# Alan-404/Conformer

Hardware: AMD Instinct MI355X
Metric: encoder audio-frames/sec (B=32,T=1000,d=512,L=16) (higher is better)
Workload: dtype f32; 1 GPU; cfg2 Conformer-L Encoder.forward: B=32/GPU, T=1000 mel frames (T'=249), d=512, 16 blocks, 8 heads, k=31, fp32, eval, random-init weights, batch-sharded replicas; per_gpu_batch=32, mel_frames=1000

## Files before the change

### conformer_amd/_lib.py

```python
from __future__ import annotations

import ctypes
import os
from ctypes import c_char_p, c_float, c_int, c_int64, c_uint64, c_void_p

_HERE = os.path.dirname(os.path.abspath(__file__))
LIB_PATH = os.environ.get("CONFORMER_AMD_LIB") or os.path.join(_HERE, "lib", "libconformer_hip.so")

_P, _I, _L, _F, _U = c_void_p, c_int, c_int64, c_float, c_uint64
ABI_VERSION = 4

SIGNATURES = {
    "cfm_version": (c_int, []),
    "cfm_abi_version": (c_int, []),
    "cfm_gemm_bias_stats_f32": (c_int, [_P, _P, _P, _P, _P, _L, _I, _I, _L, _L, _P]),
    "cfm_gemm_bias_residual_stats_f32": (c_int, [_P, _P, _P, _P, _F, _P, _P, _L, _I, _I, _L, _L, _L, _P]),
    "cfm_gemm_splitk_f32": (c_int, [_I, _P, _P, _P, _P, _F, _P, _P, _I, _L, _I, _I, _L, _L, _L, _P]),
    "cfm_gemm_lnfold_f32": (c_int, [_I, _P, _P, _I, _F, _P, _P, _P, _P, _L, _I, _I, _L, _L, _P]),
    "cfm_layernorm_fwd_stats_f32": (c_int, [_P, _P, _P, _P, _P, _L, _I, _F, _P]),
    "cfm_ffn_pack_elems": (ctypes.c_int64, [_I, _I]),
    "cfm_ffn_pack_f32": (c_int, [_P, _P, _P, _I, _I, _P]),
    "cfm_rowgemm_pack_f32": (c_int, [_P, _P, _I, _I, _I, _P]),
    "cfm_rowchain_f32": (c_int, [_I, _I, _I, _I, _P, _L, _P, _P, _P, _L, _P, _L, _P, _I, _F, _P, _P, _P, _P, _F, _I, _P, _L, _P, _P, _P, _F,
                                 _P, _P, _P, _F, _P, _L, _L, _I, _P]),
# ... 83 lines not shown
    "cfm_hotword_pack": (c_int, [_I, _P, _P, _I, _P, _P, _I, _P, _P, _P, _P, ctypes.c_size_t]),
    "cfm_hotword_count": (c_int, [_P, _P, _P, _I, ctypes.c_double, _P, _P, _P]),
    "cfm_ctc_beam_hw_workspace_bytes": (ctypes.c_size_t, [_I, _I, _I, _I]),
    "cfm_ctc_beam_hw_decode_f32": (c_int, [_P, _P, _I, _I, _I, _I, _I, _I, _F, _F, _I, _P, ctypes.c_double, ctypes.c_double,
                                           ctypes.c_double, _I, _P, ctypes.c_double, _P, ctypes.c_size_t, _P, _P, _P, _P, _P,
                                           _P]),
    "cfm_ctc_beam_stream_state_bytes": (ctypes.c_size_t, [_I, _I, _I, _I, _I, _I]),
    "cfm_ctc_beam_stream_init": (c_int, [_I, _I, _I, _I, _P, _I, _P, _P, ctypes.c_size_t, _P]),
    "cfm_ctc_beam_stream_step_f32": (c_int, [_P, _P, _I, _I, _I, _I, _I, _I, _F, _F, _I, _P, ctypes.c_double, ctypes.c_double,
                                             ctypes.c_double, _I, _P, ctypes.c_double, _P, ctypes.c_size_t, _I, _I, _P, _P, _P,
                                             _P, _P, _P]),
    "cfm_ctc_beam_stream_finish_f32": (c_int, [_I, _I, _I, _I, _P, ctypes.c_double, ctypes.c_double, ctypes.c_double, _I, _P,
                                               ctypes.c_double, _P, ctypes.c_size_t, _I, _P, _P, _P, _P, _P, _P]),
    "cfm_ctc_beam_stream_reset_slots": (c_int, [_I, _I, _I, _I, _P, _I, _P, _P, _I, _P, ctypes.c_size_t, _P]),
    "cfm_lstm_fwd_carry_f32": (c_int, [_P, _P, _P, _P, _P, _P, _P, _P, _I, _I, _I, _P]),
    "cfm_lstm_fwd_frag_carry_f32": (c_int, [_P, _P, _P, _P, _P, _P, _P, _P, _P, _I, _I, _I, _P]),
    "cfm_lstm_fwd_mfma16_carry_f32": (c_int, [_I, _P, _P, _P, _P, _P, _P, _P, _P, _P, _I, _I, _I, _P]),
    "cfm_lstm_fwd_f32": (c_int, [_P, _P, _P, _P, _P, _P, _P, _I, _I, _I, _P]),
    "cfm_lstm_fwd_frag_f32": (c_int, [_P, _P, _P, _P, _P, _P, _P, _P, _I, _I, _I, _P]),
    "cfm_lstm_bwd_frag_f32": (c_int, [_P, _P, _P, _P, _P, _P, _P, _P, _I, _I, _I, _P]),
    "cfm_debug_lstm_trace": (c_int, [_P]),
    "cfm_debug_dw16_trace": (c_int, [_P]),
    "cfm_linear_bwd_weight_mfma16_f32": (c_int, [_I, _P, _I, _L, _P, _I, _L, _P, _L, _P, _I, _I, _L, _F, _P]),
    "cfm_lstm_fwd_mfma16_f32": (c_int, [_I, _P, _P, _P, _P, _P, _P, _P, _P, _I, _I, _I, _P]),
    "cfm_lstm_bwd_mfma16_f32": (c_int, [_I, _P, _P, _P, _P, _P, _P, _P, _P, _I, _I, _I, _P]),
    "cfm_lstm_bwd_f32": (c_int, [_P, _P, _P, _P, _P, _P, _P, _I, _I, _I, _P]),
    "cfm_swish_bn_eval_f32": (c_int, [_P, _P, _P, _P, _P, _F, _P, _L, _I, _P]),
    "cfm_swish_bn_stats_f32": (c_int, [_P, _P, _P, _P, _P, _F, _L, _I, _P]),
    "cfm_swish_bn_bwd_f32": (c_int, [_P, _P, _P, _P, _P, _F, _I, _P, _P, _P, _L, _I, _P]),
    "cfm_split_pack_elems": (ctypes.c_int64, [_I, _I, _I]),
    "cfm_split_pack_bf16_f32": (c_int, [_I, _P, _P, _I, _I, _P]),
    "cfm_gemm_split_bf16_f32": (c_int, [_I, _I, _P, _P, _P, _P, _F, _P, _L, _I, _I, _L, _L, _L, _P]),
    "cfm_subsample_conv2_relu_split_bf16_f32": (c_int, [_I, _P, _P, _P, _P, _I, _I, _I, _I, _P]),
    "cfm_ctc_workspace_floats": (ctypes.c_int64, [_I, _I, _I]),
    "cfm_ctc_loss_fwd_f32": (c_int, [_P, _P, _P, _L, _L, _P, _P, _I, _I, _I, _I, _I, _P, _P, _P]),
    "cfm_ctc_loss_bwd_f32": (c_int, [_P, _P, _P, _L, _L, _P, _P, _I, _I, _I, _I, _I, _P, _P, _P, _P]),
    "cfm_ctc_align_workspace_bytes": (ctypes.c_size_t, [_I, _I, _I]),
    "cfm_ctc_align_f32": (c_int, [_P, _P, _P, _P, _I, _I, _I, _I, _I, _P, ctypes.c_size_t, _P, _P, _P, _P, _P, _P, _P, _P]),
    "cfm_relpos_attention_rows_f32": (c_int, [_P, _P, _P, _L, _P, _L, _P, _P, _P, _P, _L, _I, _I, _I, _I, _I, _I, _I, _P, _P]),
    "cfm_relpos_attention_slots_f32": (c_int, [_P, _P, _P, _L, _P, _L, _P, _P, _P, _P, _P, _P, _L, _I, _I, _I, _I, _I, _I, _P, _P]),
    "cfm_relpos_attention_slots_mfma16_f32": (c_int, [_I, _P, _P, _P, _I, _L, _P, _L, _P, _P, _P, _P, _P, _P, _L, _I, _I, _I, _I, _I, _I,
                                                      _P, _P]),
    "cfm_debug_attention_trace_f32": (c_int, [_P, _P, _P, _L, _P, _L, _P, _P, _P, _P, _L, _I, _I, _I, _I, _P, _P]),
    "cfm_debug_set_bwd_tile": (c_int, [_I]),
    "cfm_debug_set_attention_waves": (c_int, [_I]),
    "cfm_debug_gemm_cfg_f32": (c_int, [_I, _P, _P, _P, _P, _F, _P, _L, _I, _I, _P, _P]),
    "cfm_debug_set_conv2_bk": (c_int, [_I]),
    "cfm_debug_ffn_trace": (c_int, [_P, _I]),
    "cfm_debug_ffn_variant": (c_int, [_I]),
    "cfm_debug_ffn_layout": (c_int, [_I, _I]),
    "cfm_relpos_table_f32": (c_int, [_P, _P, _I, _I, _P]),
    "cfm_relpos_attention_fwd_f32": (c_int, [_P, _P, _P, _L, _P, _L, _P, _P, _P, _P, _L, _P, _I, _I, _I, _I, _P]),
    "cfm_dwconv_bn_swish_fwd_f32": (c_int, [_P, _P, _P, _P, _P, _P, _P, _F, _P, _I, _I, _I, _I, _P]),
    "cfm_subsample_conv1_relu_f32": (c_int, [_P, _P, _P, _P, _I, _I, _I, _I, _P]),
    "cfm_pack_conv2_weight_f32": (c_int, [_P, _P, _I, _P]),
    "cfm_subsample_conv2_relu_f32": (c_int, [_P, _P, _P, _P, _I, _I, _I, _I, _P]),
    "cfm_pack_linear_weight_f32": (c_int, [_P, _P, _I, _I, _I, _P]),
    "cfm_conv2_wino_plane_elems": (c_int64, [_I, _I, _I, _I]),
    "cfm_pack_conv2_wino_weight_f32": (c_int, [_P, _P, _I, _P]),
    "cfm_subsample_conv2_wino_relu_f32": (c_int, [_P, _P, _P, _P, _P, _I, _I, _I, _I, _P]),
}


class ConformerHipError(RuntimeError):
    pass


_lib = None


def load() -> ctypes.CDLL:
    global _lib
    if _lib is not None:
        return _lib
    if not os.path.exists(LIB_PATH):
        raise ConformerHipError(
            f"{LIB_PATH} is missing: build it with `python -m conformer_amd.build` "
            "(there is no CPU/eager fallback for the Conformer hot path)")
    import torch
    lib = ctypes.CDLL(LIB_PATH, mode=ctypes.RTLD_GLOBAL)
    try:
        lib.cfm_abi_version.restype = c_int
        got = int(lib.cfm_abi_version())
    except AttributeError:
        got = 0
    if got != ABI_VERSION:
        raise ConformerHipError(f"{LIB_PATH} implements C-ABI revision {got}, this binding needs {ABI_VERSION}: rebuild it with "
                                "`python -m conformer_amd.build`")
    for name, (res, args) in SIGNATURES.items():
        fn = getattr(lib, name)
        fn.restype = res
        fn.argtypes = args
    _lib = lib
    return lib


class CastItem(ctypes.Structure):
    _fields_ = [("src", ctypes.c_void_p), ("dst", ctypes.c_void_p), ("rows", ctypes.c_int64), ("cols", ctypes.c_int64),
                ("transpose", ctypes.c_int)]


CALLS = [0]


def check(status: int, what: str) -> None:
    CALLS[0] += 1
# ... 4 lines not shown
```

### conformer_amd/model/utils/convolution.py

```python
from typing import Optional, Tuple

import torch
import torch.nn as nn
import torch.nn.functional as F

from ... import autograd as ag
from ... import ops
from ._guard import PackCache, active_dropout, refuse_dropout
from .activation import GLU, Swish


class ConvolutionModule(nn.Module):
    def __init__(self, channels: int, kernel_size: int, dropout_rate: float = 0.0) -> None:
        super().__init__()
        self.layer_norm = nn.LayerNorm(normalized_shape=channels)
        self.pointwise_conv_1 = nn.Conv1d(channels, channels * 2, kernel_size=1)
        self.glu = GLU(dim=1)
        self.deepwise_conv = nn.Conv1d(channels, channels, kernel_size=kernel_size, padding=(kernel_size - 1) // 2,
                                       groups=channels)
        self.batch_norm = nn.BatchNorm1d(num_features=channels)
        self.swish = Swish()
        self.pointwise_conv_2 = nn.Conv1d(channels, channels, kernel_size=1)
        self.dropout = nn.Dropout(p=dropout_rate)
        self._packs = PackCache()

    def depthwise_eval(self, g: torch.Tensor, for_gemm: bool = False) -> torch.Tensor:
        bn = self.batch_norm
        return ops.dwconv_bn_swish(g, self.deepwise_conv.weight, self.deepwise_conv.bias, bn.weight, bn.bias,
                                   bn.running_mean, bn.running_var, bn.eps, for_gemm=for_gemm)

    def fused(self, x: torch.Tensor, residual: Optional[torch.Tensor] = None, stats: Optional[torch.Tensor] = None,
              emit_stats: bool = False, stream=None):
        refuse_dropout(self, "ConvolutionModule")
        bn = self.batch_norm
        train_bn = bn.training or bn.running_mean is None
        if train_bn and (bn.momentum is None or not bn.track_running_stats):
            raise NotImplementedError("ConvolutionModule: only the default BatchNorm1d(momentum=0.1, "
                                      "track_running_stats=True) is built")
        if train_bn and not ag.needs_grad(self, x, residual):
            h = ops.layernorm(x, self.layer_norm.weight, self.layer_norm.bias, self.layer_norm.eps, for_gemm=True)
            g = ops.linear_glu(h, self.pointwise_conv_1.weight, self.pointwise_conv_1.bias)
            bm, bv = ops.dwconv_bn_batch_stats(g, self.deepwise_conv.weight, self.deepwise_conv.bias, bn.running_mean,
                                               bn.running_var, bn.momentum)
            bn.num_batches_tracked += 1
            s = ops.dwconv_bn_swish(g, self.deepwise_conv.weight, self.deepwise_conv.bias, bn.weight, bn.bias, bm, bv,
                                    bn.eps, for_gemm=True)
            if residual is None:
                return ops.linear(s, self.pointwise_conv_2.weight, self.pointwise_conv_2.bias)
            return ops.linear_residual(s, self.pointwise_conv_2.weight, self.pointwise_conv_2.bias, residual, 1.0)
        if ag.needs_grad(self, x, residual):
            if residual is not None and residual is not x:
                raise NotImplementedError("ConvolutionModule.fused: pass residual=x (block.py:23)")
            out = ag.ConvModuleFn.apply(x, self.layer_norm.weight, self.layer_norm.bias, self.pointwise_conv_1.weight,
                                        self.pointwise_conv_1.bias, self.deepwise_conv.weight, self.deepwise_conv.bias,
                                        bn.weight, bn.bias, bn.running_mean, bn.running_var,
                                        self.pointwise_conv_2.weight, self.pointwise_conv_2.bias,
                                        self.layer_norm.eps, bn.eps, train_bn, bn.momentum if train_bn else 0.0,
                                        active_dropout(self.dropout))
            if train_bn:
                bn.num_batches_tracked += 1
            return out if residual is not None else out - x
        if stats is not None:
            ln, pw1 = self.layer_norm, self.pointwise_conv_1
            wf, bf, cs = self._packs.get("ln_fold", (pw1.weight, pw1.bias, ln.weight, ln.bias),
                                         lambda: ops.fold_layernorm(pw1.weight, pw1.bias, ln.weight, ln.bias))
            g = ops.linear_lnfold(x, stats, wf, bf, cs, ln.eps, glu=True)
        else:
            h = ops.layernorm(x, self.layer_norm.weight, self.layer_norm.bias, self.layer_norm.eps, for_gemm=stream is None)
            g = ops.linear_glu(h, self.pointwise_conv_1.weight, self.pointwise_conv_1.bias)
        s = self.depthwise_eval(g, for_gemm=True) if stream is None else stream.depthwise(self, g)
        if residual is None:
            if emit_stats:
                return ops.linear(s, self.pointwise_conv_2.weight, self.pointwise_conv_2.bias, emit_stats=True)
            return ops.linear(s, self.pointwise_conv_2.weight, self.pointwise_conv_2.bias)
        return ops.linear_residual(s, self.pointwise_conv_2.weight, self.pointwise_conv_2.bias, residual, 1.0, emit_stats=emit_stats)

    def forward(self, x: torch.Tensor) -> torch.Tensor:
        return self.fused(x)


class ConvolutionSubsampling(nn.Module):
    def __init__(self, channels: int) -> None:
        super().__init__()
        self.conv_1 = nn.Conv2d(1, channels, kernel_size=3, stride=2)
        self.act_1 = nn.ReLU()
        self.conv_2 = nn.Conv2d(channels, channels, kernel_size=3, stride=2)
        self.act_2 = nn.ReLU()
        self._packs = PackCache()

    @staticmethod
    def out_lengths(lengths: Optional[torch.Tensor]) -> Optional[torch.Tensor]:
        if lengths is None:
            return None
        if lengths.is_cuda and lengths.dtype == torch.int64:
            return ops.subsampled_lengths(lengths)
        return torch.div(torch.div(lengths - 1, 2, rounding_mode="floor") - 1, 2, rounding_mode="floor")

    def channel_last(self, x: torch.Tensor) -> torch.Tensor:
        if ag.needs_grad(self, x):
            if x.requires_grad:
                raise NotImplementedError("ConvolutionSubsampling: the gradient w.r.t. the input spectrogram is not "
                                          "built (the reference never needs it: the input is data)")
            return ag.SubsampleStemFn.apply(x, self.conv_1.weight, self.conv_1.bias, self.conv_2.weight, self.conv_2.bias)
        w2p = self._packs.get("w2p", (self.conv_2.weight,), lambda: ops.pack_conv2_weight(self.conv_2.weight))
        w2w = None
        if ops.conv2_winograd_ok(self.conv_2.weight.shape[0]):
            w2w = self._packs.get("w2w", (self.conv_2.weight,), lambda: ops.pack_conv2_wino_weight(self.conv_2.weight))
        return ops.subsample_stem(x, self.conv_1.weight, self.conv_1.bias, w2p, self.conv_2.bias, w2w=w2w)

    def forward(self, x: torch.Tensor, lengths: Optional[torch.Tensor] = None) -> Tuple[torch.Tensor, Optional[torch.Tensor]]:
        h = self.channel_last(x)
        if h.dtype != torch.float32:
            h = h.float()
        B, T2, _ = h.shape
        C = self.conv_1.out_channels
        h = h.view(B, T2, -1, C).transpose(2, 3).reshape(B, T2, -1)
        return h, self.out_lengths(lengths)


class DepthWiseSeperableConvolution(nn.Module):

    def __init__(self, in_channels: int, out_channels: int) -> None:
        super().__init__()
# ... 20 lines not shown
```

### conformer_amd/ops.py

```python
from __future__ import annotations

import threading
import ctypes
from typing import Optional, Tuple

import torch

from . import _lib
from ._derived import DerivedCache


def _stream() -> int:
    return torch.cuda.current_stream().cuda_stream


def _req(t: torch.Tensor, name: str, dtype=torch.float32) -> torch.Tensor:
    if not isinstance(t, torch.Tensor) or not t.is_cuda:
        raise _lib.ConformerHipError(
            f"{name}: expected a tensor on a HIP device, got {getattr(t, 'device', type(t))}; "
            "the Conformer hot path only exists as gfx950 kernels (no CPU fallback)")
    if t.dtype != dtype:
        raise _lib.ConformerHipError(f"{name}: expected dtype {dtype}, got {t.dtype}")
    return t if t.is_contiguous() else t.contiguous()

# ... 566 lines not shown
    _req_pos(pos, T, d)
    if not qkv.is_contiguous():
        raise _lib.ConformerHipError("relpos_attention_slots: qkv (S,T,3d) must be a contiguous cache buffer")
    if ctx is None:
        ctx = torch.empty(B, q_max, d, device=qkv.device, dtype=torch.float32)
    ctx = _req(ctx, "ctx")
    if ctx.shape != (B, q_max, d) or not ctx.is_contiguous():
        raise _lib.ConformerHipError(f"relpos_attention_slots: ctx must be a contiguous ({B},{q_max},{d}) tensor")
    lengths = _req(lengths, "lengths", torch.int64)
    q_begin = _req(q_begin, "q_begin", torch.int64)
    q_count = _req(q_count, "q_count", torch.int64)
    for name, t in (("lengths", lengths), ("q_begin", q_begin), ("q_count", q_count)):
        if t.shape != (B,) or not t.is_contiguous():
            raise _lib.ConformerHipError(f"relpos_attention_slots: {name} must be a contiguous ({B},) int64 tensor")
    nsplit = (_key_split16 if prec else _key_split)(B, n_heads, q_max, T, keys_hint)
    ws = torch.empty(nsplit * B * q_max * (d + n_heads), device=qkv.device, dtype=torch.float32) if nsplit > 1 else None
    base = qkv.data_ptr()
    if prec != PREC_F32:
        esz = 2 if q16 else 4
        st = _lib.load().cfm_relpos_attention_slots_mfma16_f32(prec, base, base + esz * d, base + 2 * esz * d, int(q16), d3,
                                                               pos.data_ptr(), pos.stride(0), u.data_ptr(), v.data_ptr(),
                                                               q_begin.data_ptr(), q_count.data_ptr(), lengths.data_ptr(),
                                                               ctx.data_ptr(), d, B, T, n_heads, d // n_heads, q_max, nsplit,
                                                               _p(ws), _stream())
        _lib.check(st, "cfm_relpos_attention_slots_mfma16_f32")
        return ctx
    st = _lib.load().cfm_relpos_attention_slots_f32(base, base + 4 * d, base + 8 * d, d3, pos.data_ptr(), pos.stride(0),
                                                    u.data_ptr(), v.data_ptr(), q_begin.data_ptr(), q_count.data_ptr(),
                                                    lengths.data_ptr(), ctx.data_ptr(), d, B, T, n_heads, d // n_heads, q_max,
                                                    nsplit, _p(ws), _stream())
    _lib.check(st, "cfm_relpos_attention_slots_f32")
    return ctx


def dwconv_bn_swish(g, w, b, bn_w, bn_b, bn_mean, bn_var, eps: float = 1e-5, for_gemm: bool = False) -> torch.Tensor:
    g = _req(g, "g"); w = _req(w, "dw weight"); b = _req(b, "dw bias")
    B, T, C = g.shape
    K = w.shape[-1]
    p16 = out16_ok(C) if for_gemm and K in (3, 7, 15, 31) else 0
    if p16:
        y = torch.empty(g.shape, device=g.device, dtype=_DT16[p16])
        st = _lib.load().cfm_dwconv_bn_swish_fwd_out16_f32(p16, g.data_ptr(), w.data_ptr(), b.data_ptr(), _req(bn_w, "bn_w").data_ptr(),
                                                           _req(bn_b, "bn_b").data_ptr(), _req(bn_mean, "bn_mean").data_ptr(),
                                                           _req(bn_var, "bn_var").data_ptr(), eps, y.data_ptr(), B, T, C, K,
                                                           _stream())
        _lib.check(st, "cfm_dwconv_bn_swish_fwd_out16_f32")
        return y
    y = _f32_like(g)
    st = _lib.load().cfm_dwconv_bn_swish_fwd_f32(g.data_ptr(), w.data_ptr(), b.data_ptr(), _req(bn_w, "bn_w").data_ptr(),
                                                 _req(bn_b, "bn_b").data_ptr(), _req(bn_mean, "bn_mean").data_ptr(),
                                                 _req(bn_var, "bn_var").data_ptr(), eps, y.data_ptr(), B, T, C, K,
                                                 _stream())
    _lib.check(st, "cfm_dwconv_bn_swish_fwd_f32")
    return y


def pack_conv2_weight(w2: torch.Tensor) -> torch.Tensor:
    w2 = _req(w2, "conv_2.weight")
    C = w2.shape[0]
    out = torch.empty(C, 9 * C, device=w2.device, dtype=torch.float32)
    _lib.check(_lib.load().cfm_pack_conv2_weight_f32(w2.data_ptr(), out.data_ptr(), C, _stream()), "cfm_pack_conv2_weight_f32")
    return out


_CONV2_WINOGRAD = __import__("os").environ.get("CONFORMER_AMD_CONV2_WINOGRAD", "1") == "1"


def set_conv2_winograd(on: bool) -> bool:
    global _CONV2_WINOGRAD
    prev, _CONV2_WINOGRAD = _CONV2_WINOGRAD, bool(on)
    return prev


def conv2_winograd_ok(C: int) -> bool:
    return bool(_CONV2_WINOGRAD and C % 256 == 0 and not mfma16_prec() and not _fp32_planes)


def pack_conv2_wino_weight(w2: torch.Tensor) -> torch.Tensor:
    w2 = _req(w2, "conv_2.weight")
    C = w2.shape[0]
    out = torch.empty(25 * C * C, device=w2.device, dtype=torch.float32)
    _lib.check(_lib.load().cfm_pack_conv2_wino_weight_f32(w2.data_ptr(), out.data_ptr(), C, _stream()),
               "cfm_pack_conv2_wino_weight_f32")
    return out


def pack_linear_weight(wl: torch.Tensor, C: int, F2: int) -> torch.Tensor:
    wl = _req(wl, "linear.weight")
    out = _f32_like(wl)
    _lib.check(_lib.load().cfm_pack_linear_weight_f32(wl.data_ptr(), out.data_ptr(), wl.shape[0], C, F2, _stream()),
               "cfm_pack_linear_weight_f32")
    return out


def subsample_stem(x: torch.Tensor, w1, b1, w2p, b2, w2w=None) -> torch.Tensor:
    x = _req(x, "x"); w1 = _req(w1, "conv_1.weight"); b1 = _req(b1, "conv_1.bias")
    w2p = _req(w2p, "packed conv_2.weight"); b2 = _req(b2, "conv_2.bias")
    B, F, T = x.shape
    C = w1.shape[0]
    F1, T1 = (F - 1) // 2, (T - 1) // 2
    F2, T2 = (F1 - 1) // 2, (T1 - 1) // 2
    lib = _lib.load()
    p16 = out16_ok(C) if C % 64 == 0 else 0
    if p16:
        h1 = torch.empty(B, T1, F1, C, device=x.device, dtype=_DT16[p16])
        _lib.check(lib.cfm_subsample_conv1_relu_out16_f32(p16, x.data_ptr(), w1.data_ptr(), b1.data_ptr(), h1.data_ptr(), B, F,
# ... 646 lines not shown
```

### include/conformer_hip.h

```cpp
#ifndef CONFORMER_HIP_H
#define CONFORMER_HIP_H

#include <stddef.h>
#include <stdint.h>

#ifdef __cplusplus
extern "C" {
#endif

typedef void* cfm_stream_t;

enum cfm_status {
    CFM_OK = 0,
    CFM_ERR_BAD_SHAPE = -1,
    CFM_ERR_UNSUPPORTED = -2,
    CFM_ERR_NULL = -3,
    CFM_ERR_LAUNCH = -4,
    CFM_ERR_DEVICE = -5,
    CFM_ERR_ALIGN = -6
};

int cfm_version(void);
int cfm_abi_version(void);
#define CFM_ABI_VERSION 4
// ... 9 lines not shown
int cfm_gemm_bias_swish_f32(const float* A, const float* W, const float* bias, float* C,
                            int64_t M, int N, int K, int64_t lda, int64_t ldc, cfm_stream_t stream);
int cfm_gemm_bias_relu_f32(const float* A, const float* W, const float* bias, float* C,
                           int64_t M, int N, int K, int64_t lda, int64_t ldc, cfm_stream_t stream);
int cfm_gemm_bias_glu_f32(const float* A, const float* W, const float* bias, float* C,
                          int64_t M, int n_out, int K, int64_t lda, int64_t ldc, cfm_stream_t stream);
int cfm_gemm_bias_residual_f32(const float* A, const float* W, const float* bias, const float* R,
                               float alpha, float* C, int64_t M, int N, int K,
                               int64_t lda, int64_t ldr, int64_t ldc, cfm_stream_t stream);

int cfm_gemm_splitk_f32(int epi, const float* A, const float* W, const float* bias, const float* R_or_null,
                        float alpha, float* C, float* workspace, int splits, int64_t M, int N, int K,
                        int64_t lda, int64_t ldr, int64_t ldc, cfm_stream_t stream);

int cfm_gemm_bias_stats_f32(const float* A, const float* W, const float* bias, float* C, float* stats_out,
                            int64_t M, int N, int K, int64_t lda, int64_t ldc, cfm_stream_t stream);
int cfm_gemm_bias_residual_stats_f32(const float* A, const float* W, const float* bias, const float* R,
                                     float alpha, float* C, float* stats_out, int64_t M, int N, int K,
                                     int64_t lda, int64_t ldr, int64_t ldc, cfm_stream_t stream);
int cfm_gemm_lnfold_f32(int epi, const float* A, const float* ln_stats, int ln_parts, float ln_eps,
                        const float* Wf, const float* bias_f, const float* colsum, float* C,
                        int64_t M, int N, int K, int64_t lda, int64_t ldc, cfm_stream_t stream);
int cfm_layernorm_fwd_stats_f32(const float* x, const float* gamma, const float* beta, float* y,
                                float* stats_out, int64_t rows, int d, float eps, cfm_stream_t stream);

int64_t cfm_ffn_pack_elems(int d, int hidden);
int cfm_ffn_pack_f32(const float* W1f, const float* W2, float* Wp, int d, int hidden, cfm_stream_t stream);
int cfm_ffn_fused_f32(const float* X, int64_t ldx, const float* ln_stats, int ln_parts, float ln_eps, const float* Wp,
                      const float* b1f, const float* colsum1, const float* b2, float alpha, float* Y, int64_t ldy,
                      int mode, float* stats_out, const float* gamma2, const float* beta2, float eps2, int64_t M,
                      int d, int hidden, cfm_stream_t stream);

int cfm_rowgemm_pack_f32(const float* W, float* Wp, int N, int d, int glu, cfm_stream_t stream);
int cfm_rowchain_f32(int pre, int core, int post, int mode, const float* X, int64_t ldx, const float* Wpre_packed,
                     const float* bpre, const float* R, int64_t ldr, float* Y1, int64_t ldy1, const float* ln_stats,
                     int ln_parts, float ln_eps, const float* Wffn_packed, const float* b1f, const float* colsum1,
                     const float* b2, float alpha, int hidden, float* Y, int64_t ldy, float* stats_out,
                     const float* gamma2, const float* beta2, float eps2, const float* Wpost_packed, const float* bpost,
                     const float* cspost, float post_eps, float* Z, int64_t ldz, int64_t M, int d, cfm_stream_t stream);
int64_t cfm_ffn_tile_stride_f4(int d);
int cfm_ffn_rotate(void);

int cfm_relpos_table_f32(const float* div_term, float* pe, int T, int d, cfm_stream_t stream);

int cfm_relpos_attention_fwd_f32(const float* q, const float* k, const float* v, int64_t ld,
                                 const float* pos, int64_t ldp, const float* u, const float* vbias,
                                 const int64_t* lengths_or_null, float* ctx, int64_t ldo,
                                 float* lse_or_null, int B, int T, int H, int dh, cfm_stream_t stream);

int cfm_dwconv_bn_swish_fwd_f32(const float* g, const float* w, const float* bias,
                                const float* bn_weight, const float* bn_bias,
                                const float* bn_mean, const float* bn_var, float bn_eps,
                                float* y, int B, int T, int C, int K, cfm_stream_t stream);

int cfm_subsample_conv1_relu_f32(const float* x, const float* w1, const float* b1, float* h1,
                                 int B, int F, int T, int C, cfm_stream_t stream);
int cfm_pack_conv2_weight_f32(const float* w2, float* w2p, int C, cfm_stream_t stream);
int cfm_subsample_conv2_relu_f32(const float* h1, const float* w2p, const float* b2, float* h2,
                                 int B, int F1, int T1, int C, cfm_stream_t stream);
int cfm_pack_linear_weight_f32(const float* wl, float* wlp, int d_out, int C, int F2, cfm_stream_t stream);
int64_t cfm_conv2_wino_plane_elems(int B, int F1, int T1, int C);
int cfm_pack_conv2_wino_weight_f32(const float* w2, float* wwp, int C, cfm_stream_t stream);
int cfm_subsample_conv2_wino_relu_f32(const float* h1, const float* wwp, const float* b2, float* planes, float* h2,
                                      int B, int F1, int T1, int C, cfm_stream_t stream);

#define CFM_PREC_F32 0
#define CFM_PREC_BF16 1
#define CFM_PREC_FP16 2
int cfm_gemm_mfma16_f32(int prec, int epi, const void* A, int a_is_16bit, const void* W, int w_is_16bit,
                        const float* bias, const float* R_or_null, float alpha, void* C, int c_is_16bit,
                        void* Z_or_null, int z_is_16bit, int64_t M, int N, int K, int64_t lda, int64_t ldr,
                        int64_t ldc, float drop_p, uint64_t drop_seed, cfm_stream_t stream);
#define CFM_CAST_BATCH 48
typedef struct cfm_cast_item {
    const float* src;
    void* dst;
    int64_t rows, cols;
    int transpose;
} cfm_cast_item;
int cfm_cast16_multi_f32(int prec, const cfm_cast_item* items, int count, cfm_stream_t stream);
int cfm_layernorm_fwd_out16_f32(int prec, const float* x, const float* gamma, const float* beta, void* y16,
                                float* mean_or_null, float* rstd_or_null, int64_t rows, int d, float eps,
                                cfm_stream_t stream);
int cfm_cast16_f32(int prec, const float* src, void* dst, int64_t n, cfm_stream_t stream);
int cfm_relpos_attention_mfma16_f32(int prec, const float* q, const float* k, const float* v, int64_t ld,
                                    const float* pos, int64_t ldp, const float* u, const float* vbias,
                                    const int64_t* lengths_or_null, float* ctx, int64_t ldo, float* lse_or_null, int B,
                                    int T, int H, int dh, float drop_p, uint64_t drop_seed, cfm_stream_t stream);
int cfm_relpos_attention_rows_mfma16_f32(int prec, const float* q, const float* k, const float* v, int64_t ld,
                                         const float* pos, int64_t ldp, const float* u, const float* vbias,
                                         const int64_t* lengths, float* ctx, int64_t ldo, int B, int T, int H, int dh,
                                         int q_begin, int q_count, cfm_stream_t stream);
int cfm_relpos_attention_io16_mfma16_f32(int prec, const void* q, const void* k, const void* v, int qkv_is_16bit, int64_t ld,
                                         const float* pos, int64_t ldp, const float* u, const float* vbias,
                                         const int64_t* lengths_or_null, void* ctx, int ctx_is_16bit, int64_t ldo, int B, int T,
                                         int H, int dh, cfm_stream_t stream);
int cfm_subsample_conv2_relu_mfma16_f32(int prec, const void* h1, int h1_is_16bit, const void* w2p, int w_is_16bit,
                                        const float* b2, void* h2, int h2_is_16bit, int B, int F1, int T1, int C,
                                        cfm_stream_t stream);
int cfm_subsample_conv1_relu_out16_f32(int prec, const float* x, const float* w1, const float* b1, void* h1, int B, int F,
                                       int T, int C, cfm_stream_t stream);
int cfm_gemm_bwd_batched_mfma16_f32(int prec, const float* A, int a_col, int64_t lda, const void* B, int b_col,
                                    int b_is_16bit, int64_t ldb, const void* Z_or_null, int z_is_16bit, int64_t ldz, float alpha, void* C,
                                    int64_t ldc, int c_is_16bit, int I, int J, int64_t Kc, int allow_split, int accumulate,
                                    int nbatch, int nb1, int64_t sa0, int64_t sa1, int64_t sb0, int64_t sb1,
                                    int64_t sc0, int64_t sc1, float drop_p, uint64_t drop_seed,
// ... 62 lines not shown
                             cfm_stream_t stream);
int cfm_layernorm_bwd_params_f32(const float* x, const float* dy, const float* mean, const float* rstd,
                                 float* dgamma, float* dbeta, int64_t rows, int d, cfm_stream_t stream);
size_t cfm_layernorm_bwd_workspace_bytes(int64_t rows, int d);
int cfm_layernorm_bwd_f32(const float* x, const float* gamma, const float* dy, const float* mean,
                          const float* rstd, const float* dres_or_null, float* dx, float* dgamma, float* dbeta,
                          int64_t rows, int d, void* workspace, size_t workspace_bytes, cfm_stream_t stream);

int cfm_colsum_f32(const float* X, int64_t ld, int64_t rows, int cols, float alpha, float* out,
                   cfm_stream_t stream);

int cfm_glu_fwd_f32(const float* z, float* y, int64_t rows, int n, cfm_stream_t stream);
int cfm_glu_bwd_f32(const float* z, const float* dy, float* dz, int64_t rows, int n, cfm_stream_t stream);

int cfm_dwconv_bn_swish_bwd_f32(const float* g, const float* dy, const float* w, const float* bias,
                                const float* bn_weight, const float* bn_bias, const float* bn_mean,
                                const float* bn_var, float bn_eps, int train_stats, float* dc_ws, float* dg,
                                float* dw, float* dbias, float* dgamma, float* dbeta, int B, int T, int C,
                                int K, cfm_stream_t stream);

size_t cfm_dwconv_bn_stats_workspace_bytes(int B, int T, int C);
int cfm_dwconv_bn_stats_f32(const float* g, const float* w, const float* bias, float* batch_mean,
                            float* batch_var, float* running_mean_or_null, float* running_var_or_null,
                            float momentum, int B, int T, int C, int K, void* workspace, size_t workspace_bytes,
                            cfm_stream_t stream);

int cfm_relpos_attention_bwd_f32(const float* q, const float* k, const float* v, int64_t ld, const float* pos,
                                 int64_t ldp, const float* u, const float* vbias, const int64_t* lengths_or_null,
                                 const float* ctx, const float* dctx, int64_t ldo, const float* lse, float* dq,
                                 float* dk, float* dv, int64_t ldg, float* dpos, int64_t lddp, float* du,
                                 float* dvbias, int B, int T, int H, int dh, float drop_p, uint64_t drop_seed,
                                 int prec, cfm_stream_t stream);

int cfm_relpos_attention_bwd_mfma16_f32(int prec, const float* q, const float* k, const float* v, int64_t ld,
                                        const float* pos, int64_t ldp, const float* u, const float* vbias,
                                        const int64_t* lengths_or_null, const float* ctx, const float* dctx, int64_t ldo,
                                        const float* lse, float* dq, float* dk, float* dv, int64_t ldg, float* dpos,
                                        int64_t lddp, float* du, float* dvbias, int B, int T, int H, int dh,
                                        float drop_p, uint64_t drop_seed, cfm_stream_t stream);

int cfm_debug_attention_bwd_trace_f32(void* trace_or_null);
int cfm_debug_attention_bwd_trace_mfma16(void* trace_or_null);
int cfm_debug_dw16_trace(void* trace_or_null);
int cfm_debug_lstm_trace(void* trace_or_null);
int cfm_debug_gemm_mfma16_force_tile(int tile);
int cfm_debug_gemm_mfma16_trace(void* trace_or_null);
int cfm_debug_gemm_last_tile(int family, int* out);

int cfm_debug_gemm_cfg_f32(int cfg, const float* A, const float* W, const float* bias, const float* R,
                           float alpha, float* C, int64_t M, int N, int K, void* trace_or_null,
                           cfm_stream_t stream);
int cfm_debug_ffn_trace(void* trace_or_null, int per_slice);
int cfm_debug_ffn_variant(int v);
int cfm_debug_ffn_layout(int pad_f4, int rotate);
int cfm_debug_set_conv2_bk(int bk);

int cfm_relu_bwd_f32(const float* y, const float* dy, float* dz, int64_t n, cfm_stream_t stream);
int cfm_subsample_conv2_bwd_weight_f32(const float* dz2, const float* h1, float* dw2p, int B, int F1, int T1,
                                       int C, cfm_stream_t stream);
int cfm_pack_conv2_weight_t_f32(const float* w2, float* w2c, int C, cfm_stream_t stream);
int cfm_subsample_conv2_bwd_input_f32(const float* dz2, const float* w2c, float* dh1, int B, int F1, int T1,
                                      int C, cfm_stream_t stream);
int cfm_subsample_conv1_bwd_f32(const float* x, const float* w1, const float* b1, const float* dh1, float* dw1,
                                float* db1, int B, int F, int T, int C, cfm_stream_t stream);

typedef struct cfm_adam_tensor {
    float* param;
    const float* grad;
    float* exp_avg;
    float* exp_avg_sq;
    int64_t numel;
} cfm_adam_tensor;
int cfm_adam_step_f32(const cfm_adam_tensor* tensors, int n_tensors, float lr, float beta1, float beta2, float eps,
                      float bias_c1, float sqrt_bias_c2, cfm_stream_t stream);
int cfm_greedy_ctc_decode_f32(const float* logits, const int64_t* lengths_or_null, int64_t* frame_ids,
                              int64_t* tokens, int64_t* counts, int B, int T, int V, int pad_id, int unk_id,
                              cfm_stream_t stream);

size_t cfm_ctc_beam_workspace_bytes(int B, int T, int W, int K);
int cfm_ctc_beam_decode_f32(const float* logits, const int64_t* lengths_or_null, int B, int T, int V, int blank_id,
                            int beam_width, int max_candidates, float token_min_logp, float beam_prune_logp, int n_best,
                            void* workspace, size_t workspace_bytes, int64_t* tokens, int64_t* counts, float* scores,
                            int64_t* num_hyps, cfm_stream_t stream);

size_t cfm_ngram_lm_pack_bytes(int order, const int64_t* ngram_counts, int n_words, int64_t word_cp_total, int V,
                               int64_t tok_cp_total);
int cfm_ngram_lm_pack(int order, const int64_t* ngram_counts, const int32_t* ngram_words, const float* ngram_logp,
                      const float* ngram_backoff, int n_words, const int64_t* word_cp_offsets, const int32_t* word_cp, int bos_id,
                      int eos_id, int unk_id, int V, const int64_t* tok_cp_offsets, const int32_t* tok_cp, const int32_t* tok_kind,
                      void* out, size_t out_bytes);
int cfm_ngram_lm_score_f64(const void* lm_tables, const int32_t* words, const int64_t* offsets, int n_sentences, int boundary,
                           double* out, cfm_stream_t stream);
size_t cfm_ctc_beam_lm_workspace_bytes(int B, int T, int W, int K);
int cfm_ctc_beam_lm_decode_f32(const float* logits, const int64_t* lengths_or_null, int B, int T, int V, int blank_id,
                               int beam_width, int max_candidates, float token_min_logp, float beam_prune_logp, int n_best,
                               const void* lm_tables, double alpha, double beta, double unk_score_offset, int score_boundary,
                               void* workspace, size_t workspace_bytes, int64_t* tokens, int64_t* counts, float* scores,
                               float* am_scores, int64_t* num_hyps, cfm_stream_t stream);

size_t cfm_hotword_pack_bytes(int n_unigrams, int64_t uni_cp_total, int n_phrases, int64_t phrase_word_total, int V,
                              int64_t tok_cp_total);
int cfm_hotword_pack(int n_unigrams, const int64_t* uni_cp_offsets, const int32_t* uni_cp, int n_phrases,
                     const int64_t* phrase_offsets, const int32_t* phrase_words, int V, const int64_t* tok_cp_offsets,
                     const int32_t* tok_cp, const int32_t* tok_kind, void* out, size_t out_bytes);
int cfm_hotword_count(const void* hw_tables, const int32_t* tokens, const int64_t* offsets, int n_seqs, double weight,
                      int32_t* counts, double* bonus, int32_t* final_counts);
// ... 117 lines not shown
```

Baseline: 1.685 million audio-frames/sec.

## Fuse LN-folded GLU pointwise GEMM with depthwise conv, BatchNorm and Swish

Adds a HIP kernel that computes the LayerNorm-folded pointwise_conv_1 GEMM with its GLU epilogue into an LDS tile spanning a full sequence chunk plus halo. It then applies the depthwise conv, eval BatchNorm and Swish directly from LDS. This is meant to remove the global write and re-read of the GLU output and one kernel launch per conformer block. In exchange the grid is one 512-thread workgroup per (batch, chunk, 64-channel group), which may give low occupancy. Halo rows are recomputed when T spans several chunks. A shape heuristic gates the path and it is on by default through an environment flag.

```diff
diff --git a/conformer_amd/_lib.py b/conformer_amd/_lib.py
--- a/conformer_amd/_lib.py
+++ b/conformer_amd/_lib.py
@@ -159,6 +159,8 @@
     "cfm_relpos_table_f32": (c_int, [_P, _P, _I, _I, _P]),
     "cfm_relpos_attention_fwd_f32": (c_int, [_P, _P, _P, _L, _P, _L, _P, _P, _P, _P, _L, _P, _I, _I, _I, _I, _P]),
     "cfm_dwconv_bn_swish_fwd_f32": (c_int, [_P, _P, _P, _P, _P, _P, _P, _F, _P, _I, _I, _I, _I, _P]),
+    "cfm_convmod_glu_dwconv_f32": (c_int, [_P, _L, _P, _I, _F, _P, _P, _P, _P, _P, _P, _P, _P, _P, _F, _P, _L, _I, _I, _I, _I, _P]),
+    "cfm_debug_convmod_variant": (c_int, [_I]),
     "cfm_subsample_conv1_relu_f32": (c_int, [_P, _P, _P, _P, _I, _I, _I, _I, _P]),
     "cfm_pack_conv2_weight_f32": (c_int, [_P, _P, _I, _P]),
     "cfm_subsample_conv2_relu_f32": (c_int, [_P, _P, _P, _P, _I, _I, _I, _I, _P]),
diff --git a/conformer_amd/csrc/convmod_fused_f32.hip b/conformer_amd/csrc/convmod_fused_f32.hip
--- /dev/null
+++ b/conformer_amd/csrc/convmod_fused_f32.hip
@@ -0,0 +1,265 @@
+#include "gemm_shared.h"
+
+namespace {
+
+#define CONVMOD_MFMA_SLICE(FA, FB)                                                                          \
+    _Pragma("unroll") for (int e = 0; e < 4; ++e)                                                           \
+    _Pragma("unroll") for (int mt = 0; mt < TM; ++mt)                                                       \
+    _Pragma("unroll") for (int nt = 0; nt < TN; ++nt)                                                       \
+        acc[mt][nt] = __builtin_amdgcn_mfma_f32_32x32x2f32(FB[nt][e], FA[mt][e], acc[mt][nt], 0, 0, 0)
+
+struct ConvModArgs {
+    GemmArgs g;
+    const float* dw_w; const float* dw_b; const float* bn_w; const float* bn_b; const float* bn_mean; const float* bn_var;
+    float bn_eps;
+    float* y; int64_t ldy;
+    int T, nchunks, ncg;
+    int variant;
+};
+
+template <int K>
+__global__ __launch_bounds__(512, 2) void convmod_fused_kernel(const ConvModArgs a) {
+    constexpr int BM = 256, BN = 128, TM = 2, TN = 2, BK = 16, LDSR = BK + 4;
+    constexpr int HALF = (K - 1) / 2, OUT = BM - (K - 1);
+    constexpr int F = EPF_INFER | EPF_LN_CONSUME;
+    constexpr int LDS_STAGE = 2 * (BM + BN) * LDSR;
+    constexpr int TP = 64 + 4;
+    constexpr int LDS_TILE = (BM + K - 1) * TP;
+    constexpr int LDS_MAIN = LDS_TILE > LDS_STAGE ? LDS_TILE : LDS_STAGE;
+    __shared__ __attribute__((aligned(16))) float lds[LDS_MAIN + 2 * BM + 64 * K];
+    float* rowstats = lds + LDS_MAIN;
+    float* taps = rowstats + 2 * BM;
+    float* As = lds;
+    float* Bs = lds + 2 * BM * LDSR;
+    float* tile = lds;
+    const GemmArgs& g = a.g;
+
+    const unsigned tl = xcd_remap(blockIdx.x, gridDim.x);
+    const int cg = (int)(tl % (unsigned)a.ncg);
+    const unsigned uc = tl / (unsigned)a.ncg;
+    const int b = (int)(uc / (unsigned)a.nchunks), ch = (int)(uc % (unsigned)a.nchunks);
+    const int f0 = ch * OUT;
+    const int64_t m0 = (int64_t)b * a.T + f0;
+    const int rows_here = min(BM, a.T - f0);
+    const int n0 = cg * 64;
+
+    const int tid = threadIdx.x, lane = tid & 63;
+    const int wave = __builtin_amdgcn_readfirstlane(tid >> 6);
+    const int wr = wave >> 1, wc = wave & 1;
+    const int li = lane & 31, hf = lane >> 5;
+
+    constexpr int CPR = BK / 4, RPP = 512 / CPR, PA = BM / RPP, PB = BN / RPP;
+    const int chunk = tid & (CPR - 1), srow = tid / CPR;
+    const float* a_ptr[PA];
+    const float* w_ptr[PB];
+#pragma unroll
+    for (int i = 0; i < PA; ++i) a_ptr[i] = g.A + (m0 + min(srow + RPP * i, rows_here - 1)) * g.lda + chunk * 4;
+#pragma unroll
+    for (int i = 0; i < PB; ++i) w_ptr[i] = w_row_ptr<EPI_GLU, BN>(g, n0, srow + RPP * i) + chunk * 4;
+
+    const int nkt = g.K / BK;
+    f32x4 ra0[PA], rb0[PB], ra1[PA], rb1[PB];
+    auto load_tile = [&](f32x4 (&ra)[PA], f32x4 (&rb)[PB], int kt) __attribute__((always_inline)) {
+        const int k = kt * BK;
+#pragma unroll
+        for (int i = 0; i < PA; ++i) ra[i] = *reinterpret_cast<const f32x4*>(a_ptr[i] + k);
+#pragma unroll
+        for (int i = 0; i < PB; ++i) rb[i] = *reinterpret_cast<const f32x4*>(w_ptr[i] + k);
+    };
+    auto store_tile = [&](const f32x4 (&ra)[PA], const f32x4 (&rb)[PB], int buf) __attribute__((always_inline)) {
+#pragma unroll
+        for (int i = 0; i < PA; ++i)
+            *reinterpret_cast<f32x4*>(As + (buf * BM + srow + RPP * i) * LDSR + chunk * 4) = ra[i];
+#pragma unroll
+        for (int i = 0; i < PB; ++i)
+            *reinterpret_cast<f32x4*>(Bs + (buf * BN + srow + RPP * i) * LDSR + chunk * 4) = rb[i];
+    };
+
+    f32x16 acc[TM][TN];
+#pragma unroll
+    for (int i = 0; i < TM; ++i)
+#pragma unroll
+        for (int j = 0; j < TN; ++j)
+#pragma unroll
+            for (int r = 0; r < 16; ++r) acc[i][j][r] = 0.f;
+
+    const int a_row = wr * (BM / 4) + li, b_row = wc * (BN / 2) + li;
+    f32x4 fa0[TM], fb0[TN], fa1[TM], fb1[TN];
+    auto read_frags = [&](f32x4 (&fa)[TM], f32x4 (&fb)[TN], int buf, int c) __attribute__((always_inline)) {
+#pragma unroll
+        for (int t = 0; t < TM; ++t)
+            fa[t] = *reinterpret_cast<const f32x4*>(As + (buf * BM + a_row + 32 * t) * LDSR + 8 * c + 4 * hf);
+#pragma unroll
+        for (int t = 0; t < TN; ++t)
+            fb[t] = *reinterpret_cast<const f32x4*>(Bs + (buf * BN + b_row + 32 * t) * LDSR + 8 * c + 4 * hf);
+    };
+
+    constexpr int LN_NL = (BM * 16 / 2 + 511) / 512;
+    f32x4 lnq[LN_NL];
+    float2 ln1 = {0.f, 0.f};
+    if (g.ln_parts >= 2) {
+        const int nf4 = rows_here * (g.ln_parts >> 1);
+        const f32x4* sp = reinterpret_cast<const f32x4*>(g.ln_stats + m0 * g.ln_parts * 2);
+#pragma unroll
+        for (int i = 0; i < LN_NL; ++i) lnq[i] = sp[min(tid + 512 * i, nf4 - 1)];
+    } else {
+        ln1 = reinterpret_cast<const float2*>(g.ln_stats)[m0 + min(tid, rows_here - 1)];
+    }
+    load_tile(ra0, rb0, 0);
+    store_tile(ra0, rb0, 0);
+    load_tile(ra1, rb1, min(1, nkt - 1));
+    load_tile(ra0, rb0, min(2, nkt - 1));
+    {
+        const float ni = (float)(g.K / g.ln_parts), inv_ni = 1.0f / ni, inv_k = 1.0f / (float)g.K;
+        if (g.ln_parts >= 2) {
+            const int lpr = g.ln_parts >> 1;
+#pragma unroll
+            for (int i = 0; i < LN_NL; ++i) {
+                const float ma = lnq[i][0] * inv_ni, mb = lnq[i][2] * inv_ni, d0 = mb - ma;
+                float mean = 0.5f * (ma + mb), m2 = lnq[i][1] + lnq[i][3] + d0 * d0 * (0.5f * ni), cnt = 2.0f * ni;
+                for (int st = 1; st < lpr; st <<= 1) {
+                    const float mo = __shfl_xor(mean, st, 64), m2o = __shfl_xor(m2, st, 64), dl = mo - mean;
+                    mean = 0.5f * (mean + mo);
+                    m2 = m2 + m2o + dl * dl * (0.5f * cnt);
+                    cnt *= 2.0f;
+                }
+                const int f = tid + 512 * i, row = f / lpr;
+                if ((f & (lpr - 1)) == 0 && row < BM) {
+                    rowstats[2 * row] = mean;
+                    rowstats[2 * row + 1] = 1.0f / sqrtf(m2 * inv_k + g.ln_eps);
+                }
+            }
+        } else if (tid < BM) {
+            rowstats[2 * tid] = ln1.x * inv_k;
+            rowstats[2 * tid + 1] = 1.0f / sqrtf(ln1.y * inv_k + g.ln_eps);
+        }
+    }
+    __syncthreads();
+    read_frags(fa0, fb0, 0, 0);
+    auto k_step = [&](int kt, f32x4 (&ra)[PA], f32x4 (&rb)[PB]) __attribute__((always_inline)) {
+        const int cur = kt & 1;
+        const bool more = kt + 1 < nkt;
+        read_frags(fa1, fb1, cur, 1);
+        __builtin_amdgcn_sched_barrier(0);
+        CONVMOD_MFMA_SLICE(fa0, fb0);
+        __builtin_amdgcn_sched_barrier(0);
+        if (more) store_tile(ra, rb, cur ^ 1);
+        load_tile(ra, rb, min(kt + 3, nkt - 1));
+        __syncthreads();
+        if (more) read_frags(fa0, fb0, cur ^ 1, 0);
+        __builtin_amdgcn_sched_barrier(0);
+        CONVMOD_MFMA_SLICE(fa1, fb1);
+        __builtin_amdgcn_sched_barrier(0);
+    };
+    int kt = 0;
+    for (; kt + 1 < nkt; kt += 2) {
+        k_step(kt, ra1, rb1);
+        k_step(kt + 1, ra0, rb0);
+    }
+    if (kt < nkt) k_step(kt, ra1, rb1);
+
+    float wt[K];
+    load_taps<K>(a.dw_w, n0, g.n_out, taps, wt);
+
+    for (int f = tid; f < (K - 1) * 64; f += 512) {
+        const int r = f >> 6;
+        tile[(r < HALF ? r : BM + r) * TP + (f & 63)] = 0.f;
+    }
+    {
+        EpiOps ob[4];
+#pragma unroll
+        for (int q = 0; q < 4; ++q) gemm_epilogue_fetch_bias<EPI_GLU, F>(g, n0 + wc * 32 + 8 * q + 4 * hf, ob[q]);
+#pragma unroll
+        for (int mt = 0; mt < TM; ++mt) {
+            const int lrow = wr * (BM / 4) + mt * 32 + li;
+            const float mean = rowstats[2 * lrow], rstd = rowstats[2 * lrow + 1];
+            const bool live = lrow < rows_here;
+#pragma unroll
+            for (int q = 0; q < 4; ++q) {
+                f32x4 av = f32x4{acc[mt][0][4 * q], acc[mt][0][4 * q + 1], acc[mt][0][4 * q + 2], acc[mt][0][4 * q + 3]};
+                f32x4 gv = f32x4{acc[mt][1][4 * q], acc[mt][1][4 * q + 1], acc[mt][1][4 * q + 2], acc[mt][1][4 * q + 3]};
+                av = (av - mean * ob[q].cs) * rstd;
+                gv = (gv - mean * ob[q].cg) * rstd;
+                f32x4 zpre;
+                const f32x4 v = gemm_epilogue_compute<EPI_GLU, F>(g, av, gv, ob[q], m0 + lrow, n0 + wc * 32 + 8 * q + 4 * hf, zpre);
+                *reinterpret_cast<f32x4*>(tile + (HALF + lrow) * TP + wc * 32 + 8 * q + 4 * hf) = live ? v : f32x4{0.f, 0.f, 0.f, 0.f};
+            }
+        }
+    }
+    __syncthreads();
+
+    constexpr int TT = 32;
+    const int c = n0 + lane;
+    const int lo0 = wave * TT;
+    const int lo_begin = ch == 0 ? 0 : HALF;
+    const int lo_end = ch == a.nchunks - 1 ? a.T - f0 : BM - HALF;
+    if (lo0 >= lo_end || lo0 + TT <= lo_begin) return;
+    float* yb = a.y + m0 * a.ldy + c;
+    if (a.variant == 1) {
+#pragma unroll 4
+        for (int o = 0; o < TT; ++o) {
+            const int lo = lo0 + o;
+            if (lo >= lo_begin && lo < lo_end) yb[(int64_t)lo * a.ldy] = tile[(HALF + lo) * TP + lane];
+        }
+        return;
+    }
+    float cacc[TT];
+    const float bi = a.dw_b[c];
+#pragma unroll
+    for (int o = 0; o < TT; ++o) cacc[o] = bi;
+    float win[TT + K - 1];
+#pragma unroll
+    for (int i = 0; i < TT + K - 1; ++i) win[i] = tile[(lo0 + i) * TP + lane];
+#pragma unroll
+    for (int o = 0; o < TT; ++o)
+#pragma unroll
+        for (int j = 0; j < K; ++j) cacc[o] = fmaf(wt[j], win[o + j], cacc[o]);
+    const float inv = 1.0f / sqrtf(a.bn_var[c] + a.bn_eps);
+    const float mu = a.bn_mean[c], ga = a.bn_w[c], be = a.bn_b[c];
+#pragma unroll
+    for (int o = 0; o < TT; ++o) {
+        const int lo = lo0 + o;
+        if (lo >= lo_begin && lo < lo_end) yb[(int64_t)lo * a.ldy] = swishf_acc((cacc[o] - mu) * inv * ga + be);
+    }
+}
+
+int g_convmod_dbg = 0;
+
+inline int convmod_chunks(int T, int K) { return T <= 256 ? 1 : 1 + (T - 256 + (256 - K)) / (257 - K); }
+
+}
+
+extern "C" int cfm_convmod_glu_dwconv_f32(const float* x, int64_t ldx, const float* ln_stats, int ln_parts, float ln_eps,
+                                          const float* Wf, const float* bias_f, const float* colsum, const float* dw_w,
+                                          const float* dw_b, const float* bn_w, const float* bn_b, const float* bn_mean,
+                                          const float* bn_var, float bn_eps, float* y, int64_t ldy, int B, int T, int C, int K,
+                                          cfm_stream_t stream) {
+    CFM_REQUIRE(x && ln_stats && Wf && bias_f && colsum && dw_w && dw_b && bn_w && bn_b && bn_mean && bn_var && y, CFM_ERR_NULL);
+    CFM_REQUIRE(B > 0 && T > 0 && C > 0 && ldx >= C && ldy >= C && ln_eps >= 0.f, CFM_ERR_BAD_SHAPE);
+    CFM_REQUIRE(K == 31 || K == 15 || K == 7 || K == 3, CFM_ERR_UNSUPPORTED);
+    CFM_REQUIRE(C == 64 || C == 128 || C == 256 || C == 512, CFM_ERR_UNSUPPORTED);
+    CFM_REQUIRE(ln_parts >= 1 && C % ln_parts == 0, CFM_ERR_BAD_SHAPE);
+    CFM_REQUIRE(ln_parts <= 16 && (ln_parts & (ln_parts - 1)) == 0, CFM_ERR_UNSUPPORTED);
+    CFM_REQUIRE((ldx & 3) == 0 && CFM_ALIGNED16(x) && CFM_ALIGNED16(Wf) && CFM_ALIGNED16(bias_f) && CFM_ALIGNED16(colsum),
+                CFM_ERR_ALIGN);
+    CFM_REQUIRE((reinterpret_cast<uintptr_t>(ln_stats) & (ln_parts >= 2 ? 15u : 7u)) == 0, CFM_ERR_ALIGN);
+    CFM_REQUIRE((reinterpret_cast<uintptr_t>(y) & 3u) == 0, CFM_ERR_ALIGN);
+    ConvModArgs a{};
+    a.g.A = x; a.g.W = Wf; a.g.bias = bias_f; a.g.M = (int64_t)B * T; a.g.N = 2 * C; a.g.K = C; a.g.n_out = C; a.g.lda = ldx;
+    a.g.alpha = 1.f; a.g.ln_stats = ln_stats; a.g.ln_parts = ln_parts; a.g.ln_eps = ln_eps; a.g.ln_colsum = colsum;
+    a.dw_w = dw_w; a.dw_b = dw_b; a.bn_w = bn_w; a.bn_b = bn_b; a.bn_mean = bn_mean; a.bn_var = bn_var; a.bn_eps = bn_eps;
+    a.y = y; a.ldy = ldy; a.T = T; a.nchunks = convmod_chunks(T, K); a.ncg = C / 64; a.variant = g_convmod_dbg;
+    const int64_t nwg = (int64_t)B * a.nchunks * a.ncg;
+    CFM_REQUIRE(nwg < ((int64_t)1 << 31), CFM_ERR_BAD_SHAPE);
+    hipStream_t s = static_cast<hipStream_t>(stream);
+    const dim3 grid((unsigned)nwg), block(512);
+    switch (K) {
+        case 31: hipLaunchKernelGGL(convmod_fused_kernel<31>, grid, block, 0, s, a); break;
+        case 15: hipLaunchKernelGGL(convmod_fused_kernel<15>, grid, block, 0, s, a); break;
+        case 7: hipLaunchKernelGGL(convmod_fused_kernel<7>, grid, block, 0, s, a); break;
+        default: hipLaunchKernelGGL(convmod_fused_kernel<3>, grid, block, 0, s, a);
+    }
+    return cfm_launch_status();
+}
+
+extern "C" int cfm_debug_convmod_variant(int v) { const int p = g_convmod_dbg; g_convmod_dbg = v; return p; }
diff --git a/conformer_amd/model/utils/convolution.py b/conformer_amd/model/utils/convolution.py
--- a/conformer_amd/model/utils/convolution.py
+++ b/conformer_amd/model/utils/convolution.py
@@ -64,11 +64,18 @@
             ln, pw1 = self.layer_norm, self.pointwise_conv_1
             wf, bf, cs = self._packs.get("ln_fold", (pw1.weight, pw1.bias, ln.weight, ln.bias),
                                          lambda: ops.fold_layernorm(pw1.weight, pw1.bias, ln.weight, ln.bias))
-            g = ops.linear_lnfold(x, stats, wf, bf, cs, ln.eps, glu=True)
+            dw = self.deepwise_conv
+            if stream is None and x.dim() == 3 and ops.convmod_fused_ok(x.shape[0], x.shape[1], x.shape[2], dw.weight.shape[-1]):
+                g = None
+                s = ops.convmod_glu_dwconv(x, stats, wf, bf, cs, ln.eps, dw.weight, dw.bias, bn.weight, bn.bias, bn.running_mean,
+                                           bn.running_var, bn.eps)
+            else:
+                g = ops.linear_lnfold(x, stats, wf, bf, cs, ln.eps, glu=True)
         else:
             h = ops.layernorm(x, self.layer_norm.weight, self.layer_norm.bias, self.layer_norm.eps, for_gemm=stream is None)
             g = ops.linear_glu(h, self.pointwise_conv_1.weight, self.pointwise_conv_1.bias)
-        s = self.depthwise_eval(g, for_gemm=True) if stream is None else stream.depthwise(self, g)
+        if g is not None:
+            s = self.depthwise_eval(g, for_gemm=True) if stream is None else stream.depthwise(self, g)
         if residual is None:
             if emit_stats:
                 return ops.linear(s, self.pointwise_conv_2.weight, self.pointwise_conv_2.bias, emit_stats=True)
diff --git a/conformer_amd/ops.py b/conformer_amd/ops.py
--- a/conformer_amd/ops.py
+++ b/conformer_amd/ops.py
@@ -642,6 +642,52 @@
                                                  _req(bn_var, "bn_var").data_ptr(), eps, y.data_ptr(), B, T, C, K,
                                                  _stream())
     _lib.check(st, "cfm_dwconv_bn_swish_fwd_f32")
+    return y
+
+
+_CONVMOD_FUSED = __import__("os").environ.get("CONFORMER_AMD_CONVMOD_FUSED", "1") != "0"
+_CONVMOD_MIN_ROW_EFF = 0.875
+
+
+def set_convmod_fused(on: bool) -> bool:
+    global _CONVMOD_FUSED
+    prev, _CONVMOD_FUSED = _CONVMOD_FUSED, bool(on)
+    return prev
+
+
+def convmod_chunks(T: int, K: int) -> int:
+    return 1 if T <= 256 else 1 + (T - 256 + (256 - K)) // (257 - K)
+
+
+def convmod_fused_ok(B: int, T: int, C: int, K: int) -> bool:
+    if not (_CONVMOD_FUSED and ln_fold_ok(C) and C % 64 == 0 and K in (3, 7, 15, 31) and B > 0 and T > 0):
+        return False
+    chunks = convmod_chunks(T, K)
+    blocks = B * chunks * (C // 64)
+    rounds = (blocks + 255) // 256
+    return blocks >= 0.9 * 256 * rounds and T >= _CONVMOD_MIN_ROW_EFF * 256 * chunks
+
+
+def convmod_glu_dwconv(x, stats, wf, bf, cs, ln_eps: float, w, b, bn_w, bn_b, bn_mean, bn_var, bn_eps: float = 1e-5) -> torch.Tensor:
+    x = _req(x, "x"); stats = _req(stats, "ln_stats"); wf = _req(wf, "Wf"); bf = _req(bf, "bias_f"); cs = _req(cs, "colsum")
+    w = _req(w, "dw weight"); b = _req(b, "dw bias")
+    if x.dim() != 3:
+        raise _lib.ConformerHipError(f"convmod_glu_dwconv: x must be (B, T, C), got {tuple(x.shape)}")
+    B, T, C = x.shape
+    K = w.shape[-1]
+    if (tuple(wf.shape) != (2 * C, C) or stats.dim() != 3 or stats.shape[0] != B * T or stats.shape[2] != 2 or w.numel() != C * K
+            or bf.numel() != 2 * C or cs.numel() != 2 * C or b.numel() != C):
+        raise _lib.ConformerHipError(f"convmod_glu_dwconv: x{tuple(x.shape)}, Wf{tuple(wf.shape)}, stats{tuple(stats.shape)}, "
+                                     f"dw weight{tuple(w.shape)} do not match")
+    bn = [_req(t, n) for t, n in ((bn_w, "bn_w"), (bn_b, "bn_b"), (bn_mean, "bn_mean"), (bn_var, "bn_var"))]
+    if any(t.numel() != C for t in bn):
+        raise _lib.ConformerHipError(f"convmod_glu_dwconv: the BatchNorm tensors must have {C} values")
+    y = torch.empty(B, T, C, device=x.device, dtype=torch.float32)
+    if B * T:
+        _lib.check(_lib.load().cfm_convmod_glu_dwconv_f32(x.data_ptr(), C, stats.data_ptr(), stats.shape[1], float(ln_eps), wf.data_ptr(),
+                                                          bf.data_ptr(), cs.data_ptr(), w.data_ptr(), b.data_ptr(), bn[0].data_ptr(),
+                                                          bn[1].data_ptr(), bn[2].data_ptr(), bn[3].data_ptr(), float(bn_eps),
+                                                          y.data_ptr(), C, B, T, C, K, _stream()), "cfm_convmod_glu_dwconv_f32")
     return y
 
 
diff --git a/include/conformer_hip.h b/include/conformer_hip.h
--- a/include/conformer_hip.h
+++ b/include/conformer_hip.h
@@ -85,6 +85,12 @@
                                 const float* bn_weight, const float* bn_bias,
                                 const float* bn_mean, const float* bn_var, float bn_eps,
                                 float* y, int B, int T, int C, int K, cfm_stream_t stream);
+
+int cfm_convmod_glu_dwconv_f32(const float* x, int64_t ldx, const float* ln_stats, int ln_parts, float ln_eps,
+                               const float* Wf, const float* bias_f, const float* colsum, const float* dw_w,
+                               const float* dw_b, const float* bn_w, const float* bn_b, const float* bn_mean,
+                               const float* bn_var, float bn_eps, float* y, int64_t ldy, int B, int T, int C, int K,
+                               cfm_stream_t stream);
 
 int cfm_subsample_conv1_relu_f32(const float* x, const float* w1, const float* b1, float* h1,
                                  int B, int F, int T, int C, cfm_stream_t stream);
@@ -253,6 +259,7 @@
                            cfm_stream_t stream);
 int cfm_debug_ffn_trace(void* trace_or_null, int per_slice);
 int cfm_debug_ffn_variant(int v);
+int cfm_debug_convmod_variant(int v);
 int cfm_debug_ffn_layout(int pad_f4, int rotate);
 int cfm_debug_set_conv2_bk(int bk);
 
```

After: 1.706 million audio-frames/sec, median of 6. 1.01x the previous value.
